# cloneofsimo/paint-with-words-sd

Measured on AMD Instinct MI355X. Metric: 512x512 images/sec (30 steps, CFG) SD1.5+PwW, higher is better.
Workload: dtype bf16

## Files before the change

paint-with-words-sd_amd/csrc/pww_conv.hip:

```cpp
#include "pww_common.h"

namespace pww {

namespace {

constexpr int CV_BM = 128, CV_THREADS = 256;

__device__ __forceinline__ f32x4 mfma16(f16x8 a, f16x8 b, f32x4 c) { return __builtin_amdgcn_mfma_f32_16x16x32_f16(a, b, c, 0, 0, 0); }
__device__ __forceinline__ f32x4 mfma16(bf16x8 a, bf16x8 b, f32x4 c) { return __builtin_amdgcn_mfma_f32_16x16x32_bf16(a, b, c, 0, 0, 0); }

struct ConvCold {
    const void *bias, *residual;
    int nsplit, nslab;
};

__device__ __forceinline__ int xcd_remap(int orig, int nwg) {
    const int xcd = orig & 7, q = nwg >> 3, r = nwg & 7;
    return (xcd < r ? xcd * (q + 1) : r * (q + 1) + (xcd - r) * q) + (orig >> 3);
}

template <typename T>
__device__ __forceinline__ void epilogue4(const f32x4 &a, const ConvCold &cold, T *y, long off, int n) {
    typedef typename Vec<T>::v4 V4;
    V4 o;
#pragma unroll
    for (int j = 0; j < 4; ++j) o[j] = (T)a[j];
    if (cold.bias) {
        const V4 b = *reinterpret_cast<const V4 *>(reinterpret_cast<const T *>(cold.bias) + n);
#pragma unroll
        for (int j = 0; j < 4; ++j) o[j] = (T)((float)o[j] + (float)b[j]);
    }
    if (cold.residual) {
        const V4 r = *reinterpret_cast<const V4 *>(reinterpret_cast<const T *>(cold.residual) + off);
#pragma unroll
        for (int j = 0; j < 4; ++j) o[j] = (T)((float)r[j] + (float)o[j]);
    }
    *reinterpret_cast<V4 *>(y + off) = o;
}

template <typename T, int BN, bool SPLIT>
__global__ void __launch_bounds__(CV_THREADS) conv3x3_kernel(const T *__restrict__ x, const T *__restrict__ w, void *__restrict__ out, int M, int N,
                                                            int Cin, int Hin, int Win, int Wo, int HWo, const ConvCold cold) {
    typedef typename Vec<T>::v8 V8;
    constexpr int BM = CV_BM, XL = BM * 8 / CV_THREADS, WL = BN * 8 / CV_THREADS, RM = 4, RN = BN / 32;
    constexpr int XBYTES = BM * 128, STAGE = (BM + BN) * 128;
    __shared__ __attribute__((aligned(16))) char lds[2 * STAGE];

    const int geo = cold.nslab >> 24;
    const int nslab = cold.nslab & 0xffffff;
    const int stride = geo & 15, up = geo >> 4;
    const int Hv = Hin << up, Wv = Win << up;
    const int tid = threadIdx.x, lane = tid & 63, wave = tid >> 6, wm = wave >> 1, wn = wave & 1;
    const int ntm = (M + BM - 1) / BM;
    const int bid = xcd_remap(blockIdx.x, gridDim.x);
    const int tile = SPLIT ? bid / cold.nsplit : bid, ks = SPLIT ? bid % cold.nsplit : 0;
    const int tm = tile % ntm, tn = tile / ntm;
    const int s_begin = SPLIT ? (int)((long)ks * nslab / cold.nsplit) : 0;
    const int s_end = SPLIT ? (int)((long)(ks + 1) * nslab / cold.nsplit) : nslab;
    const int K9 = 9 * Cin;

    const int c = tid & 7;
    int pix[XL], y0[XL], x0[XL];
#pragma unroll
    for (int i = 0; i < XL; ++i) {
        int m = tm * BM + (tid >> 3) + 32 * i;
        m = m < M ? m : M - 1;
        const int b = m / HWo, rem = m - b * HWo, oy = rem / Wo, ox = rem - oy * Wo;
        pix[i] = b * Hin * Win;
        y0[i] = oy * stride - 1;
        x0[i] = ox * stride - 1;
    }
    const T *wrow = w + (long)(tn * BN + (tid >> 3)) * K9 + c * 8;
    const int swz = ((c ^ ((tid >> 3) & 7)) << 4);

    u32x4 xr[XL], wr[WL];
    unsigned xok = 0;
    int tap = s_begin / (Cin >> 6), ci0 = (s_begin - tap * (Cin >> 6)) << 6;
    auto load = [&](int s) {
        const int ky = tap / 3, kx = tap - ky * 3;
#pragma unroll
        for (int i = 0; i < XL; ++i) {
            const int iyv = y0[i] + ky, ixv = x0[i] + kx;
            const bool ok = (unsigned)iyv < (unsigned)Hv && (unsigned)ixv < (unsigned)Wv;
            const int iy = ok ? iyv >> up : 0, ix = ok ? ixv >> up : 0;
            xr[i] = *reinterpret_cast<const u32x4 *>(x + (unsigned)((pix[i] + iy * Win + ix) * Cin + ci0 + c * 8));
            xok = (xok & ~(1u << i)) | ((unsigned)ok << i);
        }
#pragma unroll
        for (int j = 0; j < WL; ++j) wr[j] = *reinterpret_cast<const u32x4 *>(wrow + (long)(32 * j) * K9 + s * 64);
        ci0 += 64;
        if (ci0 == Cin) { ci0 = 0; ++tap; }
    };
    auto store = [&](int buf) {
        char *base = lds + buf * STAGE;
#pragma unroll
        for (int i = 0; i < XL; ++i) {
            const u32x4 z = {0u, 0u, 0u, 0u};
            *reinterpret_cast<u32x4 *>(base + ((tid >> 3) + 32 * i) * 128 + swz) = (xok >> i) & 1u ? xr[i] : z;
        }
#pragma unroll
        for (int j = 0; j < WL; ++j) *reinterpret_cast<u32x4 *>(base + XBYTES + ((tid >> 3) + 32 * j) * 128 + swz) = wr[j];
    };

    f32x4 acc[RN][RM];
#pragma unroll
    for (int r = 0; r < RN; ++r)
#pragma unroll
        for (int i = 0; i < RM; ++i) acc[r][i] = f32x4{0.f, 0.f, 0.f, 0.f};

    const int fr = lane & 15, fq = lane >> 4;
    if (s_begin < s_end) {
        load(s_begin);
        store(0);
        __syncthreads();
    }
    for (int s = s_begin; s < s_end; ++s) {
        const int cur = (s - s_begin) & 1;
        if (s + 1 < s_end) load(s + 1);
        const char *bx = lds + cur * STAGE, *bw = bx + XBYTES;
#pragma unroll
        for (int kk = 0; kk < 2; ++kk) {
            V8 xf[RM], wf[RN];
#pragma unroll
            for (int i = 0; i < RM; ++i) {
                const int row = wm * 64 + i * 16 + fr;
                xf[i] = *reinterpret_cast<const V8 *>(bx + row * 128 + (((kk * 4 + fq) ^ (row & 7)) << 4));
            }
#pragma unroll
            for (int r = 0; r < RN; ++r) {
                const int row = wn * (BN / 2) + r * 16 + fr;
                wf[r] = *reinterpret_cast<const V8 *>(bw + row * 128 + (((kk * 4 + fq) ^ (row & 7)) << 4));
            }
#pragma unroll
            for (int r = 0; r < RN; ++r)
#pragma unroll
                for (int i = 0; i < RM; ++i) acc[r][i] = mfma16(wf[r], xf[i], acc[r][i]);
        }
        if (s + 1 < s_end) store(cur ^ 1);
        __syncthreads();
    }

#pragma unroll
    for (int i = 0; i < RM; ++i) {
        const int m = tm * BM + wm * 64 + i * 16 + fr;
        if (m >= M) continue;
#pragma unroll
        for (int r = 0; r < RN; ++r) {
            const int n = tn * BN + wn * (BN / 2) + r * 16 + fq * 4;
            if (SPLIT) *reinterpret_cast<f32x4 *>(reinterpret_cast<float *>(out) + ((long)ks * M + m) * N + n) = acc[r][i];
            else epilogue4<T>(acc[r][i], cold, reinterpret_cast<T *>(out), (long)m * N + n, n);
        }
    }
}

template <typename T>
__global__ void __launch_bounds__(256) conv3x3_fold_kernel(const float *__restrict__ ws, T *__restrict__ y, long n4, int N, long MN, const ConvCold cold) {
    const long q = (long)blockIdx.x * 256 + threadIdx.x;
    if (q >= n4) return;
    const long off = q * 4;
    f32x4 a = *reinterpret_cast<const f32x4 *>(ws + off);
    for (int s = 1; s < cold.nsplit; ++s) a += *reinterpret_cast<const f32x4 *>(ws + s * MN + off);
    epilogue4<T>(a, cold, y, off, (int)(off % N));
}

struct ConvTune { int M, N, nslab, bn, nsplit; };
constexpr ConvTune CONV_TUNED[] = {
    {8192, 320, 45, 64, 2}, {8192, 320, 90, 64, 4}, {8192, 320, 135, 64, 3}, {8192, 640, 90, 128, 3},
    {2048, 320, 45, 64, 6}, {2048, 640, 45, 64, 3}, {2048, 640, 90, 128, 6}, {2048, 640, 135, 128, 6}, {2048, 640, 180, 128, 6},
    {2048, 640, 270, 128, 6}, {2048, 1280, 180, 128, 3},
    {512, 640, 90, 64, 6}, {512, 1280, 90, 64, 6}, {512, 1280, 180, 128, 12}, {512, 1280, 270, 128, 12}, {512, 1280, 360, 128, 12},
    {128, 1280, 180, 64, 12}, {128, 1280, 360, 64, 24},
    {65536, 640, 90, 128, 1}, {16384, 1280, 180, 128, 1},
    {4096, 640, 90, 128, 3}, {4096, 1280, 90, 128, 3}, {4096, 1280, 180, 128, 3}, {4096, 1280, 270, 128, 3}, {4096, 1280, 360, 128, 3},
    {1024, 1280, 180, 128, 6}, {1024, 1280, 360, 128, 6},
};

struct ConvPlan {
    int M, Ho, Wo, bn, nsplit, nslab, ntiles;
};

bool plan_conv(const pww_conv_desc_t *d, ConvPlan *p) {
    if (!d || d->size < sizeof(pww_conv_desc_t)) { set_error("conv3x3: descriptor missing or older than this library (size %u)", d ? d->size : 0u); return false; }
    const int up = d->upsample, s = d->stride;
    if ((d->dtype != PWW_DTYPE_F16 && d->dtype != PWW_DTYPE_BF16) || d->B < 1 || d->Hin < 1 || d->Win < 1 || d->Cin < 64 || d->Cin % 64 != 0
        || d->Cout < 64 || d->Cout % 64 != 0 || (s != 1 && s != 2) || (up != 0 && up != 1) || (up && s != 1) || d->Cin > 65536 || d->Cout > 65536) {
        set_error("conv3x3: unsupported (dtype %d B %d %dx%d Cin %d Cout %d stride %d upsample %d): Cin and Cout multiples of 64, stride 1 or 2, "
                  "upsample only at stride 1", d->dtype, d->B, d->Hin, d->Win, d->Cin, d->Cout, s, up);
        return false;
    }
    const int Hv = d->Hin << up, Wv = d->Win << up;
    p->Ho = (Hv - 1) / s + 1;
    p->Wo = (Wv - 1) / s + 1;
    const long M = (long)d->B * p->Ho * p->Wo;
    if ((long)d->B * d->Hin * d->Win * d->Cin >= (1L << 31) || M * d->Cout >= (1L << 31)) { set_error("conv3x3: tensor of 2^31 elements or more"); return false; }
    p->M = (int)M;
    p->nslab = 9 * d->Cin / 64;
    const ConvTune *tuned = nullptr;
    for (const ConvTune &t : CONV_TUNED)
        if (t.M == p->M && t.N == d->Cout && t.nslab == p->nslab) tuned = &t;
    p->bn = d->tile_n ? d->tile_n : tuned ? tuned->bn : (d->Cout % 128 == 0 ? 128 : 64);
    if ((p->bn != 64 && p->bn != 128) || d->Cout % p->bn != 0) { set_error("conv3x3: tile_n %d does not divide Cout %d", d->tile_n, d->Cout); return false; }
    p->ntiles = (p->M + CV_BM - 1) / CV_BM * (d->Cout / p->bn);
    int ns = d->splitk;
    if (ns <= 0 && tuned && p->bn == tuned->bn) ns = tuned->nsplit;
    if (ns <= 0) {
        ns = (480 + p->ntiles / 2) / p->ntiles;
        if (ns > p->nslab / 8) ns = p->nslab / 8;
        if (ns < 1) ns = 1;
    }
    if (ns > p->nslab || ns > 64) { set_error("conv3x3: split %d exceeds the %d K-slabs (or 64)", ns, p->nslab); return false; }
    p->nsplit = ns;
    return true;
}

template <typename T>
int conv_launch(const ConvPlan &p, const pww_conv_desc_t *d, const void *x, const void *w, const void *bias, const void *residual, void *y, void *ws,
                hipStream_t stream) {
    ConvCold cold{bias, residual, p.nsplit, p.nslab | ((d->stride | (d->upsample << 4)) << 24)};
    const T *xt = static_cast<const T *>(x), *wt = static_cast<const T *>(w);
    const int N = d->Cout, HWo = p.Ho * p.Wo;
    const dim3 grid(p.ntiles * p.nsplit), block(CV_THREADS);
    if (p.nsplit == 1) {
        if (p.bn == 128) launch_timed(conv3x3_kernel<T, 128, false>, grid, block, 0, stream, xt, wt, y, p.M, N, d->Cin, d->Hin, d->Win, p.Wo, HWo, cold);
        else launch_timed(conv3x3_kernel<T, 64, false>, grid, block, 0, stream, xt, wt, y, p.M, N, d->Cin, d->Hin, d->Win, p.Wo, HWo, cold);
        return check_hip(hipGetLastError(), "conv3x3 launch");
    }
    if (p.bn == 128) launch_timed(conv3x3_kernel<T, 128, true>, grid, block, 0, stream, xt, wt, ws, p.M, N, d->Cin, d->Hin, d->Win, p.Wo, HWo, cold);
    else launch_timed(conv3x3_kernel<T, 64, true>, grid, block, 0, stream, xt, wt, ws, p.M, N, d->Cin, d->Hin, d->Win, p.Wo, HWo, cold);
    const long MN = (long)p.M * N, n4 = MN / 4;
    launch_timed(conv3x3_fold_kernel<T>, dim3((unsigned)((n4 + 255) / 256)), dim3(256), 0, stream, static_cast<const float *>(ws), static_cast<T *>(y), n4,
                 N, MN, cold);
    return check_hip(hipGetLastError(), "conv3x3 fold launch");
}

bool al16(const void *a) { return (reinterpret_cast<uintptr_t>(a) & 15) == 0; }

}

size_t conv3x3_workspace_bytes(const pww_conv_desc_t *d) {
    ConvPlan p;
    if (!plan_conv(d, &p)) return 0;
    return p.nsplit > 1 ? (size_t)p.nsplit * p.M * d->Cout * sizeof(float) : 0;
}

int conv3x3_fwd(const void *x, const void *w, const void *bias, const void *residual, void *y, const pww_conv_desc_t *d, void *workspace,
                size_t workspace_bytes, hipStream_t stream) {
    ConvPlan p;
    if (!plan_conv(d, &p)) return PWW_ENOTSUP;
    if (!x || !w || !y) { set_error("conv3x3: x, w and y are required"); return PWW_EINVAL; }
    if (!al16(x) || !al16(w) || !al16(y) || (reinterpret_cast<uintptr_t>(bias) & 7) || (reinterpret_cast<uintptr_t>(residual) & 7)) {
        set_error("conv3x3: x, w, y must be 16-byte aligned, bias and residual 8-byte aligned");
        return PWW_EINVAL;
    }
    if (p.nsplit > 1 && (!workspace || !al16(workspace) || workspace_bytes < (size_t)p.nsplit * p.M * d->Cout * sizeof(float))) {
        set_error("conv3x3: split %d needs a 16-byte aligned workspace of %zu bytes (got %zu)", p.nsplit, (size_t)p.nsplit * p.M * d->Cout * sizeof(float),
                  workspace_bytes);
        return PWW_EINVAL;
    }
    if (!arch_ok()) return PWW_ENOTSUP;
    if (d->dtype == PWW_DTYPE_F16) return conv_launch<f16>(p, d, x, w, bias, residual, y, workspace, stream);
    return conv_launch<bf16>(p, d, x, w, bias, residual, y, workspace, stream);
}

}
```

Baseline: 4.938.

## Deepen conv3x3 global prefetch to two register stages and merge split variants

Restructures the implicit-GEMM conv3x3 main loop so global loads run two K-slabs ahead in register buffers, while LDS stays double-buffered. This hides more global memory latency. It also merges the split and non-split kernel templates into one with a runtime branch, adds an occupancy hint of 2 blocks per CU to launch_bounds, replaces per-slab weight index math with an incrementing pointer, and retunes two split and tile table entries. In exchange, the doubled register staging raises register pressure, and the runtime split check replaces a compile-time specialization.

```diff
diff --git a/paint-with-words-sd_amd/csrc/pww_conv.hip b/paint-with-words-sd_amd/csrc/pww_conv.hip
--- a/paint-with-words-sd_amd/csrc/pww_conv.hip
+++ b/paint-with-words-sd_amd/csrc/pww_conv.hip
@@ -5,6 +5,7 @@
 namespace {
 
 constexpr int CV_BM = 128, CV_THREADS = 256;
+constexpr int CV_PF = 2;
 
 __device__ __forceinline__ f32x4 mfma16(f16x8 a, f16x8 b, f32x4 c) { return __builtin_amdgcn_mfma_f32_16x16x32_f16(a, b, c, 0, 0, 0); }
 __device__ __forceinline__ f32x4 mfma16(bf16x8 a, bf16x8 b, f32x4 c) { return __builtin_amdgcn_mfma_f32_16x16x32_bf16(a, b, c, 0, 0, 0); }
@@ -38,11 +39,11 @@
     *reinterpret_cast<V4 *>(y + off) = o;
 }
 
-template <typename T, int BN, bool SPLIT>
-__global__ void __launch_bounds__(CV_THREADS) conv3x3_kernel(const T *__restrict__ x, const T *__restrict__ w, void *__restrict__ out, int M, int N,
+template <typename T, int BN>
+__global__ void __launch_bounds__(CV_THREADS, 2) conv3x3_kernel(const T *__restrict__ x, const T *__restrict__ w, void *__restrict__ out, int M, int N,
                                                             int Cin, int Hin, int Win, int Wo, int HWo, const ConvCold cold) {
     typedef typename Vec<T>::v8 V8;
-    constexpr int BM = CV_BM, XL = BM * 8 / CV_THREADS, WL = BN * 8 / CV_THREADS, RM = 4, RN = BN / 32;
+    constexpr int BM = CV_BM, PF = CV_PF, XL = BM * 8 / CV_THREADS, WL = BN * 8 / CV_THREADS, RM = 4, RN = BN / 32;
     constexpr int XBYTES = BM * 128, STAGE = (BM + BN) * 128;
     __shared__ __attribute__((aligned(16))) char lds[2 * STAGE];
 
@@ -53,10 +54,10 @@
     const int tid = threadIdx.x, lane = tid & 63, wave = tid >> 6, wm = wave >> 1, wn = wave & 1;
     const int ntm = (M + BM - 1) / BM;
     const int bid = xcd_remap(blockIdx.x, gridDim.x);
-    const int tile = SPLIT ? bid / cold.nsplit : bid, ks = SPLIT ? bid % cold.nsplit : 0;
+    const bool split = cold.nsplit > 1;
+    const int tile = bid / cold.nsplit, ks = bid - tile * cold.nsplit;
     const int tm = tile % ntm, tn = tile / ntm;
-    const int s_begin = SPLIT ? (int)((long)ks * nslab / cold.nsplit) : 0;
-    const int s_end = SPLIT ? (int)((long)(ks + 1) * nslab / cold.nsplit) : nslab;
+    const int s_begin = (int)((long)ks * nslab / cold.nsplit), s_end = (int)((long)(ks + 1) * nslab / cold.nsplit);
     const int K9 = 9 * Cin;
 
     const int c = tid & 7;
@@ -73,33 +74,36 @@
     const T *wrow = w + (long)(tn * BN + (tid >> 3)) * K9 + c * 8;
     const int swz = ((c ^ ((tid >> 3) & 7)) << 4);
 
-    u32x4 xr[XL], wr[WL];
-    unsigned xok = 0;
+    u32x4 xr[PF][XL], wr[PF][WL];
+    unsigned xok[PF];
     int tap = s_begin / (Cin >> 6), ci0 = (s_begin - tap * (Cin >> 6)) << 6;
-    auto load = [&](int s) {
+    const T *wnext = wrow + s_begin * 64;
+    auto load = [&](int p) {
         const int ky = tap / 3, kx = tap - ky * 3;
+        xok[p] = 0;
 #pragma unroll
         for (int i = 0; i < XL; ++i) {
             const int iyv = y0[i] + ky, ixv = x0[i] + kx;
             const bool ok = (unsigned)iyv < (unsigned)Hv && (unsigned)ixv < (unsigned)Wv;
             const int iy = ok ? iyv >> up : 0, ix = ok ? ixv >> up : 0;
-            xr[i] = *reinterpret_cast<const u32x4 *>(x + (unsigned)((pix[i] + iy * Win + ix) * Cin + ci0 + c * 8));
-            xok = (xok & ~(1u << i)) | ((unsigned)ok << i);
-        }
-#pragma unroll
-        for (int j = 0; j < WL; ++j) wr[j] = *reinterpret_cast<const u32x4 *>(wrow + (long)(32 * j) * K9 + s * 64);
+            xr[p][i] = *reinterpret_cast<const u32x4 *>(x + (unsigned)((pix[i] + iy * Win + ix) * Cin + ci0 + c * 8));
+            xok[p] |= (unsigned)ok << i;
+        }
+#pragma unroll
+        for (int j = 0; j < WL; ++j) wr[p][j] = *reinterpret_cast<const u32x4 *>(wnext + (long)(32 * j) * K9);
+        wnext += 64;
         ci0 += 64;
         if (ci0 == Cin) { ci0 = 0; ++tap; }
     };
-    auto store = [&](int buf) {
+    auto store = [&](int p, int buf) {
         char *base = lds + buf * STAGE;
 #pragma unroll
         for (int i = 0; i < XL; ++i) {
             const u32x4 z = {0u, 0u, 0u, 0u};
-            *reinterpret_cast<u32x4 *>(base + ((tid >> 3) + 32 * i) * 128 + swz) = (xok >> i) & 1u ? xr[i] : z;
-        }
-#pragma unroll
-        for (int j = 0; j < WL; ++j) *reinterpret_cast<u32x4 *>(base + XBYTES + ((tid >> 3) + 32 * j) * 128 + swz) = wr[j];
+            *reinterpret_cast<u32x4 *>(base + ((tid >> 3) + 32 * i) * 128 + swz) = (xok[p] >> i) & 1u ? xr[p][i] : z;
+        }
+#pragma unroll
+        for (int j = 0; j < WL; ++j) *reinterpret_cast<u32x4 *>(base + XBYTES + ((tid >> 3) + 32 * j) * 128 + swz) = wr[p][j];
     };
 
     f32x4 acc[RN][RM];
@@ -109,22 +113,15 @@
         for (int i = 0; i < RM; ++i) acc[r][i] = f32x4{0.f, 0.f, 0.f, 0.f};
 
     const int fr = lane & 15, fq = lane >> 4;
-    if (s_begin < s_end) {
-        load(s_begin);
-        store(0);
-        __syncthreads();
-    }
-    for (int s = s_begin; s < s_end; ++s) {
-        const int cur = (s - s_begin) & 1;
-        if (s + 1 < s_end) load(s + 1);
-        const char *bx = lds + cur * STAGE, *bw = bx + XBYTES;
+    auto compute = [&](int buf) {
+        const char *bx = lds + buf * STAGE, *bw = bx + XBYTES;
 #pragma unroll
         for (int kk = 0; kk < 2; ++kk) {
             V8 xf[RM], wf[RN];
 #pragma unroll
-            for (int i = 0; i < RM; ++i) {
-                const int row = wm * 64 + i * 16 + fr;
-                xf[i] = *reinterpret_cast<const V8 *>(bx + row * 128 + (((kk * 4 + fq) ^ (row & 7)) << 4));
+            for (int q = 0; q < RM; ++q) {
+                const int row = wm * 64 + q * 16 + fr;
+                xf[q] = *reinterpret_cast<const V8 *>(bx + row * 128 + (((kk * 4 + fq) ^ (row & 7)) << 4));
             }
 #pragma unroll
             for (int r = 0; r < RN; ++r) {
@@ -134,10 +131,35 @@
 #pragma unroll
             for (int r = 0; r < RN; ++r)
 #pragma unroll
-                for (int i = 0; i < RM; ++i) acc[r][i] = mfma16(wf[r], xf[i], acc[r][i]);
-        }
-        if (s + 1 < s_end) store(cur ^ 1);
-        __syncthreads();
+                for (int q = 0; q < RM; ++q) acc[r][q] = mfma16(wf[r], xf[q], acc[r][q]);
+        }
+    };
+
+    const int n = s_end - s_begin;
+    load(0);
+#pragma unroll
+    for (int p = 1; p < PF; ++p)
+        if (p < n) load(p);
+    store(0, 0);
+    __syncthreads();
+    int i = 0;
+    for (; i + 2 * PF <= n; i += PF) {
+#pragma unroll
+        for (int p = 0; p < PF; ++p) {
+            load(p);
+            compute((i + p) & 1);
+            store((p + 1) % PF, (i + p + 1) & 1);
+            __syncthreads();
+        }
+    }
+#pragma unroll
+    for (int t = 0; t < 2 * PF - 1; ++t) {
+        if (i + t < n) {
+            if (i + t + PF < n) load(t % PF);
+            compute((i + t) & 1);
+            if (i + t + 1 < n) store((t + 1) % PF, (i + t + 1) & 1);
+            __syncthreads();
+        }
     }
 
 #pragma unroll
@@ -147,7 +169,7 @@
 #pragma unroll
         for (int r = 0; r < RN; ++r) {
             const int n = tn * BN + wn * (BN / 2) + r * 16 + fq * 4;
-            if (SPLIT) *reinterpret_cast<f32x4 *>(reinterpret_cast<float *>(out) + ((long)ks * M + m) * N + n) = acc[r][i];
+            if (split) *reinterpret_cast<f32x4 *>(reinterpret_cast<float *>(out) + ((long)ks * M + m) * N + n) = acc[r][i];
             else epilogue4<T>(acc[r][i], cold, reinterpret_cast<T *>(out), (long)m * N + n, n);
         }
     }
@@ -165,10 +187,10 @@
 
 struct ConvTune { int M, N, nslab, bn, nsplit; };
 constexpr ConvTune CONV_TUNED[] = {
-    {8192, 320, 45, 64, 2}, {8192, 320, 90, 64, 4}, {8192, 320, 135, 64, 3}, {8192, 640, 90, 128, 3},
+    {8192, 320, 45, 64, 3}, {8192, 320, 90, 64, 4}, {8192, 320, 135, 64, 3}, {8192, 640, 90, 128, 3},
     {2048, 320, 45, 64, 6}, {2048, 640, 45, 64, 3}, {2048, 640, 90, 128, 6}, {2048, 640, 135, 128, 6}, {2048, 640, 180, 128, 6},
     {2048, 640, 270, 128, 6}, {2048, 1280, 180, 128, 3},
-    {512, 640, 90, 64, 6}, {512, 1280, 90, 64, 6}, {512, 1280, 180, 128, 12}, {512, 1280, 270, 128, 12}, {512, 1280, 360, 128, 12},
+    {512, 640, 90, 64, 6}, {512, 1280, 90, 128, 6}, {512, 1280, 180, 128, 12}, {512, 1280, 270, 128, 12}, {512, 1280, 360, 128, 12},
     {128, 1280, 180, 64, 12}, {128, 1280, 360, 64, 24},
     {65536, 640, 90, 128, 1}, {16384, 1280, 180, 128, 1},
     {4096, 640, 90, 128, 3}, {4096, 1280, 90, 128, 3}, {4096, 1280, 180, 128, 3}, {4096, 1280, 270, 128, 3}, {4096, 1280, 360, 128, 3},
@@ -220,13 +242,10 @@
     const T *xt = static_cast<const T *>(x), *wt = static_cast<const T *>(w);
     const int N = d->Cout, HWo = p.Ho * p.Wo;
     const dim3 grid(p.ntiles * p.nsplit), block(CV_THREADS);
-    if (p.nsplit == 1) {
-        if (p.bn == 128) launch_timed(conv3x3_kernel<T, 128, false>, grid, block, 0, stream, xt, wt, y, p.M, N, d->Cin, d->Hin, d->Win, p.Wo, HWo, cold);
-        else launch_timed(conv3x3_kernel<T, 64, false>, grid, block, 0, stream, xt, wt, y, p.M, N, d->Cin, d->Hin, d->Win, p.Wo, HWo, cold);
-        return check_hip(hipGetLastError(), "conv3x3 launch");
-    }
-    if (p.bn == 128) launch_timed(conv3x3_kernel<T, 128, true>, grid, block, 0, stream, xt, wt, ws, p.M, N, d->Cin, d->Hin, d->Win, p.Wo, HWo, cold);
-    else launch_timed(conv3x3_kernel<T, 64, true>, grid, block, 0, stream, xt, wt, ws, p.M, N, d->Cin, d->Hin, d->Win, p.Wo, HWo, cold);
+    void *out = p.nsplit == 1 ? y : ws;
+    if (p.bn == 128) launch_timed(conv3x3_kernel<T, 128>, grid, block, 0, stream, xt, wt, out, p.M, N, d->Cin, d->Hin, d->Win, p.Wo, HWo, cold);
+    else launch_timed(conv3x3_kernel<T, 64>, grid, block, 0, stream, xt, wt, out, p.M, N, d->Cin, d->Hin, d->Win, p.Wo, HWo, cold);
+    if (p.nsplit == 1) return check_hip(hipGetLastError(), "conv3x3 launch");
     const long MN = (long)p.M * N, n4 = MN / 4;
     launch_timed(conv3x3_fold_kernel<T>, dim3((unsigned)((n4 + 255) / 256)), dim3(256), 0, stream, static_cast<const float *>(ws), static_cast<T *>(y), n4,
                  N, MN, cold);
```

After: 5.023, median of 6. 1.7% higher.
